# enkeejunior1/Diffusion-Pullback

Measured on AMD Instinct MI355X. Metric: pullback top-k SVD iters/sec (SD-v1.5 mid-block, 4x64x64), higher is better.
Workload: dtype bf16; 1 GPU; BASELINE configs[2]: SD-v1.5 4x64x64 latent, no edit prompt (seeded null ctx[1,77,768]), mid-block h[1280,8,8], t=696.27; pca_rank=5, ctx=null, samples_total=5, samples_this_rank=5, samples_advanced_together=1, spectrum=shaped (configs.Spectrum()), parallelism=single process, no collective, rccl_world_size=0, repeats=7

## Files before the change

diffusion_pullback_amd/csrc/engine.cpp:

```cpp
#include <math.h>
#include <stdarg.h>
#include <stdio.h>
#include <stdlib.h>
#include <string.h>

#include <string>
#include <vector>

#include "../../include/dpb.h"
#include "kernels.h"

namespace dpb {

static thread_local char g_err[1024] = "";
void set_error(const char* fmt, ...) {
  va_list ap;
  va_start(ap, fmt);
  vsnprintf(g_err, sizeof(g_err), fmt, ap);
  va_end(ap);
}
const char* last_error() { return g_err; }

static inline size_t align_up(size_t v, size_t a = 256) { return (v + a - 1) / a * a; }
static inline int round8(int v) { return (v + 7) / 8 * 8; }
// ... 1077 lines not shown
  int n = b.kind == DPB_BUF_SHARED ? 1 : e->cur_batch;
  if (n < 1) return fail("no primal state to read (dpb_forward invalidates it; run dpb_primal first)");
  return launch_nhwc_to_nchw(e->dtype, e->P(buf), out, n, channels, b.rows, b.C, e->stream);
}

static int jvp_pass(dpb_engine* e, int src, int tap, const float* V, int nt, float* U) {
  if (!e || !V) return fail("null argument");
  if (int r = check_pair(e, src, tap, nt)) return r;
  e->n_launch = 0; e->flops = 0; e->gbytes = 0;
  const Buf& bx = e->bufs[src];
  e->n_launch++;
  if (int r = launch_nchw_to_nhwc(e->dtype, V, e->T(src), nt, seed_channels(e, src), bx.rows, bx.C, e->stream)) return r;
  if (e->tstats_bytes && !gn_deterministic()) DPB_CHECK(hipMemsetAsync(e->ws + e->tstats_off, 0, e->tstats_bytes, e->stream));
  const int last = e->producer[tap];
  std::fill(e->skip.begin(), e->skip.end(), 0);
  e->cur_tap = tap; e->pend.on = false;
  for (int i = e->producer[src] + 1; i <= last; ++i) {
    if (!e->oact[i] || e->skip[i]) continue;
    if (int r = run_op(e, e->ops[i], MODE_TANGENT, nt)) return r;
  }
  if (int r = flush_pending(e)) return r;
  if (!U) return 0;
  const Buf& bt = e->bufs[tap];
  e->n_launch++;
  return launch_nhwc_to_nchw(e->dtype, e->T(tap), U, nt, bt.Cv, bt.rows, bt.C, e->stream);
}

int dpb_jvp(dpb_engine* e, int tap, const float* V, int nt, float* U) {
  if (!U) return fail("null argument");
  return jvp_pass(e, e ? e->x_buf : -1, tap, V, nt, U);
}

int dpb_jvp_between(dpb_engine* e, int src_buf, int dst_buf, const float* V, int nt, float* U) {
  if (!e || !U) return fail("null argument");
  return jvp_pass(e, src_buf, dst_buf, V, nt, U);
}

static int vjp_pass(dpb_engine* e, int src, int tap, const float* U, int nt, float* W) {
  if (!e || !W) return fail("null argument");
  if (int r = check_pair(e, src, tap, nt)) return r;
  e->n_launch = 0; e->flops = 0; e->gbytes = 0;
  const Buf& bt = e->bufs[tap];
  std::fill(e->ginit.begin(), e->ginit.end(), 0);
  for (auto& b : e->bufs) b.g_off = b.g_off0;
  if (U) {
    e->n_launch++;
    if (int r = launch_nchw_to_nhwc(e->dtype, U, e->G(tap), nt, bt.Cv, bt.rows, bt.C, e->stream)) return r;
  } else {
    e->bufs[tap].g_off = e->bufs[tap].t_off;
  }
  e->ginit[tap] = 1;
  if (e->tstats_bytes && !gn_deterministic()) DPB_CHECK(hipMemsetAsync(e->ws + e->tstats_off, 0, e->tstats_bytes, e->stream));
  e->cur_tap = tap; e->pend.on = false;
  for (int i = e->producer[tap]; i > e->producer[src]; --i) {
    const Op& op = e->ops[i];
    if (!e->oact[i] || !e->ginit[op.d.out]) continue;
    if (int r = run_op(e, op, MODE_ADJOINT, nt)) return r;
  }
  if (int r = flush_pending(e)) return r;
  if (!e->ginit[src]) {
    for (auto& b : e->bufs) b.g_off = b.g_off0;
    return src == e->x_buf ? fail("tap buffer %d is not connected to x", tap) : fail("dst buffer %d is not connected to source buffer %d", tap, src);
  }
  const Buf& bx = e->bufs[src];
  e->n_launch++;
  const int r = launch_nhwc_to_nchw(e->dtype, e->G(src), W, nt, seed_channels(e, src), bx.rows, bx.C, e->stream);
  for (auto& b : e->bufs) b.g_off = b.g_off0;
  return r;
}

int dpb_vjp(dpb_engine* e, int tap, const float* U, int nt, float* W) {
  if (!U) return fail("null argument");
  return vjp_pass(e, e ? e->x_buf : -1, tap, U, nt, W);
}

int dpb_vjp_between(dpb_engine* e, int src_buf, int dst_buf, const float* U, int nt, float* W) {
  if (!e || !U) return fail("null argument");
  return vjp_pass(e, src_buf, dst_buf, U, nt, W);
}

int dpb_orth(const float* W, const float* Vprev, float* V, float* s, float* conv, void* scratch, int k, int64_t N, void* stream) {
  if (!W || !Vprev || !V || !s || !conv || !scratch) return fail("null argument");
  OrthArgs a;
  a.W = W; a.Vprev = Vprev; a.V = V; a.s = s; a.conv = conv; a.scratch = (double*)scratch; a.k = k; a.N = N;
  a.scratch_bytes = orth_scratch_bytes(k, N);
  return launch_orth(a, (hipStream_t)stream);
}

int dpb_orth_checked(const float* W, const float* Vprev, float* V, float* s, float* conv, void* scratch, size_t scratch_bytes, int k, int64_t N,
                     void* stream) {
  if (!W || !Vprev || !V || !s || !conv || !scratch) return fail("null argument");
  if (k < 1 || k > ORTH_MAX_RANK || N < 1) return fail("dpb_orth: k=%d outside [1,%d] or N=%lld < 1", k, ORTH_MAX_RANK, (long long)N);
  const size_t need = orth_scratch_bytes(k, N);
  if (scratch_bytes < need) return fail("dpb_orth: scratch of %zu bytes, dpb_orth_scratch_bytes(%d, %lld) = %zu", scratch_bytes, k, (long long)N, need);
  OrthArgs a;
  a.W = W; a.Vprev = Vprev; a.V = V; a.s = s; a.conv = conv; a.scratch = (double*)scratch; a.k = k; a.N = N;
  a.scratch_bytes = scratch_bytes;
  return launch_orth(a, (hipStream_t)stream);
}

size_t dpb_orth_scratch_bytes(int k, int64_t N) { return (k < 1 || k > ORTH_MAX_RANK || N < 1) ? 0 : orth_scratch_bytes(k, N); }

size_t dpb_pca_scratch_bytes(int q, int64_t N, int64_t D) { return pca_scratch_bytes(q, N, D); }

int dpb_pca_lowrank(const float* H, int64_t N, int64_t D, const float* R, int q, int niter, float* u, float* s, void* scratch,
                    size_t scratch_bytes, void* stream) {
  if (!H || !R || !u || !s || (!scratch && scratch_bytes)) return fail("dpb_pca_lowrank: null argument");
  return launch_pca_lowrank(H, N, D, R, q, niter, u, s, scratch, scratch_bytes, (hipStream_t)stream);
}

static int g_iter_alias = getenv("DPB_ITER_ALIAS") ? atoi(getenv("DPB_ITER_ALIAS")) : 1;
static int g_orth_batch = getenv("DPB_ORTH_BATCH") ? atoi(getenv("DPB_ORTH_BATCH")) : 1;
static int g_graph_iterate = 0;

static int iterate_pass(dpb_engine* e, int src, int tap, float* V, float* U, float* s, float* conv, int k, int n_iters, float* Wm, char* orth_scratch,
                        size_t orth_stride) {
  const int B = e->cur_batch;
  const int nt = k * B;
  const long N = (long)e->bufs[src].rows * seed_channels(e, src);
  long launches = 0; double fl = 0, gb = 0;
  const bool alias_ok = e->bufs[tap].Cv == e->bufs[tap].C && g_iter_alias;
  auto body = [&](bool want_u) -> int {
    const bool keep = alias_ok && !want_u;
    if (int r = jvp_pass(e, src, tap, V, nt, keep ? nullptr : U)) return r;
    launches += e->n_launch; fl += e->flops; gb += e->gbytes;
    if (int r = vjp_pass(e, src, tap, keep ? nullptr : U, nt, Wm)) return r;
    launches += e->n_launch; fl += e->flops; gb += e->gbytes;
    {
      OrthArgs a;
      a.W = Wm; a.Vprev = V; a.V = V; a.s = s; a.conv = conv; a.scratch = (double*)orth_scratch; a.k = k; a.N = N;
      a.scratch_bytes = orth_scratch_bytes(k, N);
      a.batch = B; a.stride_w = (long)k * N; a.stride_v = (long)k * N; a.stride_s = k; a.stride_conv = 2; a.scratch_stride = orth_stride;
      if (g_orth_batch) {
        if (int r = launch_orth(a, e->stream)) return r;
      } else {
        a.batch = 1;
        for (int b = 0; b < B; ++b) {
          if (int r = launch_orth(a, e->stream)) return r;
          a.W += a.stride_w; a.Vprev += a.stride_v; a.V += a.stride_v; a.s += k; a.conv += 2; a.scratch += orth_stride / sizeof(double);
        }
      }
    }
    launches += g_orth_batch ? 4 : 4 * B;
    return 0;
  };
  int it = 0;
  if (g_graph_iterate && !e->profiling && e->stream != 0 && src == e->x_buf) {
    const dpb_engine::GraphKey key{tap, k, B, V, U, s, conv};
    if (!e->gexec || !(key == e->gkey)) {
      if (int r = body(true)) return r;
      ++it;
      if (e->gexec) { (void)hipGraphExecDestroy(e->gexec); e->gexec = nullptr; }
      hipGraph_t g = nullptr;
      const long l0 = launches; const double f0 = fl, b0 = gb;
      DPB_CHECK(hipStreamBeginCapture(e->stream, hipStreamCaptureModeThreadLocal));
      const int r = body(true);
      const hipError_t ce = hipStreamEndCapture(e->stream, &g);
      e->g_launches = launches - l0; e->g_flops = fl - f0; e->g_bytes = gb - b0;
      launches = l0; fl = f0; gb = b0;
      if (r) { if (g) (void)hipGraphDestroy(g); return r; }
      DPB_CHECK(ce);
      DPB_CHECK(hipGraphInstantiate(&e->gexec, g, nullptr, nullptr, 0));
      (void)hipGraphDestroy(g);
      e->gkey = key;
    }
    for (; it < n_iters; ++it) {
      DPB_CHECK(hipGraphLaunch(e->gexec, e->stream));
      launches += e->g_launches; fl += e->g_flops; gb += e->g_bytes;
    }
  }
  for (; it < n_iters; ++it)
    if (int r = body(it == n_iters - 1)) return r;
  e->n_launch = launches; e->flops = fl; e->gbytes = gb;
  return 0;
}

int dpb_pullback_iterate(dpb_engine* e, int tap, float* V, float* U, float* s, float* conv, int k, int n_iters) {
  if (!e || !V || !U || !s || !conv) return fail("null argument");
  if (k < 1 || k > ORTH_MAX_RANK) return fail("pca_rank k=%d outside [1,%d]", k, ORTH_MAX_RANK);
  const int B = e->cur_batch;
  if (int r = check_tap(e, tap, k * (B > 0 ? B : 1))) return r;
  return iterate_pass(e, e->x_buf, tap, V, U, s, conv, k, n_iters, (float*)(e->ws + e->pbW), e->ws + e->orth, e->orth_stride);
}

static size_t between_scratch_bytes(const dpb_engine* e, int src, int k, int batch) {
  const long N = (long)e->bufs[src].rows * seed_channels(e, src);
  return align_up((size_t)batch * k * N * sizeof(float)) + (size_t)batch * align_up(orth_scratch_bytes(k, N));
}

size_t dpb_pullback_scratch_bytes(const dpb_engine* e, int src_buf, int k) {
  if (!e || k < 1 || k > ORTH_MAX_RANK || src_buf < 0 || src_buf >= (int)e->bufs.size() || e->bufs[src_buf].kind != DPB_BUF_ACT) return 0;
  return between_scratch_bytes(e, src_buf, k, e->maxB);
}

int dpb_pullback_iterate_between(dpb_engine* e, int src_buf, int dst_buf, float* V, float* U, float* s, float* conv, int k, int n_iters, void* scratch,
                                 size_t scratch_bytes) {
  if (!e || !V || !U || !s || !conv || !scratch) return fail("null argument");
  if (k < 1 || k > ORTH_MAX_RANK) return fail("pca_rank k=%d outside [1,%d]", k, ORTH_MAX_RANK);
  const int B = e->cur_batch;
  if (int r = check_pair(e, src_buf, dst_buf, k * (B > 0 ? B : 1))) return r;
  if ((uintptr_t)scratch % 256) return fail("scratch must be 256-byte aligned");
  const size_t need = between_scratch_bytes(e, src_buf, k, B);
  if (scratch_bytes < need) return fail("scratch of %zu bytes, the iteration needs %zu (dpb_pullback_scratch_bytes)", scratch_bytes, need);
  const long N = (long)e->bufs[src_buf].rows * seed_channels(e, src_buf);
  const size_t wbytes = align_up((size_t)B * k * N * sizeof(float));
  return iterate_pass(e, src_buf, dst_buf, V, U, s, conv, k, n_iters, (float*)scratch, (char*)scratch + wbytes, align_up(orth_scratch_bytes(k, N)));
}

int dpb_ddim_step(const float* x, const float* eps, float* out, float* x0, int64_t n, float a_t, float a_next, void* stream) {
  if (!x || !eps || !out) return fail("null argument");
  return launch_ddim_step(x, eps, out, x0, n, a_t, a_next, (hipStream_t)stream);
}

int dpb_embed_tokens(const int32_t* ids, const void* tok_table, const void* pos_table, int dtype, float* out, int batch, int tokens,
                     int channels, int vocab, void* stream) {
  if (!ids || !tok_table || !pos_table || !out) return fail("null argument");
  if (dtype != DPB_F32 && dtype != DPB_BF16 && dtype != DPB_F16) return fail("bad dtype %d", dtype);
  return launch_embed_tokens(dtype, ids, tok_table, pos_table, out, batch, tokens, channels, vocab, (hipStream_t)stream);
}

int dpb_lincomb(const float* x, const float* y, const float* z, float* out, int64_t n, float a, float b, float c, void* stream) {
  if (!x || !y || !out) return fail("null argument");
  return launch_lincomb(x, y, z, out, n, a, b, c, (hipStream_t)stream);
}

int dpb_engine_profile(dpb_engine* e, int enable) {
  if (!e) return fail("null engine");
  for (auto& p : e->prof) { (void)hipEventDestroy(p.a); (void)hipEventDestroy(p.b); }
  e->prof.clear();
  e->profiling = enable != 0;
  if (e->profiling) {
    hipEvent_t a, b;
    DPB_CHECK(hipEventCreate(&a));
    DPB_CHECK(hipEventCreate(&b));
    float best = 1e9f;
    for (int i = 0; i < 24; ++i) {
      DPB_CHECK(hipEventRecord(a, e->stream));
      if (int r = launch_axpy(e->dtype, e->ws + e->zeros, e->ws + e->zeros, 64, 0, e->stream)) return r;
      DPB_CHECK(hipEventRecord(b, e->stream));
      DPB_CHECK(hipEventSynchronize(b));
      float ms = 0;
      DPB_CHECK(hipEventElapsedTime(&ms, a, b));
      if (i >= 4) best = ms < best ? ms : best;
    }
    (void)hipEventDestroy(a);
    (void)hipEventDestroy(b);
    best -= 1.5e-3f;
    if (best < 0.f) best = 0.f;
    e->prof_overhead_ms = best < 1e8f ? best : 0.f;
  }
  return 0;
}

int dpb_engine_profile_dump(dpb_engine* e, const char* path) {
  if (!e || !path) return fail("null argument");
  DPB_CHECK(hipStreamSynchronize(e->stream));
  FILE* f = fopen(path, "w");
  if (!f) return fail("cannot open %s", path);
  fprintf(f, "idx,big,gather,M,N,K,Z,us,tflops,raw_us,bracket_overhead_us\n");
  int i = 0;
  for (auto& p : e->prof) {
    float raw = 0;
    (void)hipEventElapsedTime(&raw, p.a, p.b);
    const float ms = raw > e->prof_overhead_ms ? raw - e->prof_overhead_ms : 0.f;
    fprintf(f, "%d,%d,%d,%d,%d,%d,%d,%.2f,%.2f,%.2f,%.2f\n", i++, p.big, p.gather, p.M, p.N, p.K, p.Z, ms * 1e3, ms > 0 ? p.flops / (ms * 1e-3) / 1e12 : 0.0,
            raw * 1e3, e->prof_overhead_ms * 1e3);
  }
  fclose(f);
  return 0;
}

int dpb_engine_profile_read(dpb_engine* e, int big_tile, int64_t* count, double* total_ms, double* flops) {
  if (!e || !count || !total_ms || !flops) return fail("null argument");
  DPB_CHECK(hipStreamSynchronize(e->stream));
  *count = 0; *total_ms = 0; *flops = 0;
  const bool raw = big_tile >= 1000;
  if (raw) big_tile -= 1000;
  if (big_tile < 0 || big_tile > 12) return fail("dpb_engine_profile_read: kind must be 0..12 or 1000..1012");
  for (auto& p : e->prof) {
    if (p.big != big_tile) continue;
    float ms = 0;
    DPB_CHECK(hipEventElapsedTime(&ms, p.a, p.b));
    if (!raw) ms = ms > e->prof_overhead_ms ? ms - e->prof_overhead_ms : 0.f;
    *count += 1; *total_ms += ms; *flops += p.flops;
  }
  return 0;
}

int dpb_engine_profile_overhead(const dpb_engine* e, double* bracket_overhead_ms) {
  if (!e || !bracket_overhead_ms) return fail("null argument");
  *bracket_overhead_ms = e->prof_overhead_ms;
  return 0;
}

int dpb_debug_set(const char* key, int value) {
  static int tile = 0, splitk = 0, kch = 0;
  if (!key) return fail("null key");
  if (!strcmp(key, "gemm_tile")) tile = value;
  else if (!strcmp(key, "gemm_splitk")) splitk = value;
  else if (!strcmp(key, "gemm_kch")) kch = value;
  else if (!strcmp(key, "gemm_dma_auto")) { gemm_debug_dma_auto(value); return 0; }
  else if (!strcmp(key, "gemm_order")) { gemm_debug_order(value); return 0; }
  else if (!strcmp(key, "p8")) { gemm_debug_p8(value); return 0; }
  else if (!strcmp(key, "wres")) { gemm_debug_wres(value); return 0; }
  else if (!strcmp(key, "gn_deterministic")) { gn_debug_deterministic(value); return 0; }
  else if (!strcmp(key, "graph_iterate")) { g_graph_iterate = value; return 0; }
  else if (!strcmp(key, "attn_shared")) { attn_debug_shared(value); return 0; }
  else if (!strcmp(key, "lazy_reduce")) { g_lazy_reduce = value; return 0; }
  else if (!strcmp(key, "ln_fuse")) { g_ln_fuse = value; return 0; }
  else if (!strcmp(key, "cross_primal")) { g_cross_primal = value; return 0; }
  else if (!strcmp(key, "geglu_fwd")) { g_geglu_fwd = value; return 0; }
  else if (!strcmp(key, "iter_alias")) { g_iter_alias = value; return 0; }
  else return fail("unknown debug key %s", key);
  gemm_debug_set(tile, splitk, kch);
  return 0;
}

int dpb_debug_gemm_plan(int dtype, int M, int N, int K, int conv_hw, int conv_cin, int epilogue, int64_t slab_bytes, int* kind, int* tile,
                        int* splitk) {
  if (!kind || !tile || !splitk) return fail("null argument");
  if (dtype != DPB_F32 && dtype != DPB_BF16 && dtype != DPB_F16) return fail("bad dtype %d", dtype);
  static char dummy[16];
  GemmArgs a;
  a.M = M; a.N = N; a.K = K; a.lda = K; a.ldb = K; a.ldc = N;
  a.zeros = dummy;
  if (slab_bytes > 0) { a.slab = (float*)dummy; a.slab_bytes = (size_t)slab_bytes; }
  a.epi = epilogue;
  if (conv_hw > 0) {
    if (conv_cin <= 0 || K != 9 * conv_cin || M % (conv_hw * conv_hw)) return fail("conv plan: K must be 9*cin and M whole images");
    a.gather = GATHER_CONV; a.H = a.W = a.Ho = a.Wo = conv_hw; a.Cin = conv_cin; a.KS = 3; a.stride = 1; a.pad = 1; a.lda = conv_cin;
  }
  const GemmPlan pl = gemm_plan(dtype, a);
  if (pl.kind < 0) return -1;
  *kind = pl.kind; *tile = pl.tile; *splitk = pl.splitk;
  return 0;
}

int dpb_engine_stats(const dpb_engine* e, int64_t* launches, double* gemm_flops, double* gemm_bytes) {
  if (!e) return fail("null engine");
  if (launches) *launches = e->n_launch;
  if (gemm_flops) *gemm_flops = e->flops;
  if (gemm_bytes) *gemm_bytes = e->gbytes;
  return 0;
}

}
```

diffusion_pullback_amd/csrc/gemm_halo.hip:

```cpp
#include "epilogue.h"

namespace dpb {

typedef __attribute__((address_space(3))) void lds_void_t;
typedef __attribute__((address_space(1))) const void gbl_void_t;

__device__ inline bf16x8 halo_lds_read(unsigned addr) {
  bf16x8 v;
  asm volatile("ds_read_b128 %0, %1" : "=v"(v) : "v"(addr));
  return v;
}
__device__ inline void halo_wait_frags4(bf16x8 (&a)[2], bf16x8 (&b)[2]) {
  asm volatile("s_waitcnt lgkmcnt(4)" : "+v"(a[0]), "+v"(a[1]), "+v"(b[0]), "+v"(b[1]));
}
__device__ inline void halo_wait_frags0(bf16x8 (&a)[2], bf16x8 (&b)[2]) {
  asm volatile("s_waitcnt lgkmcnt(0)" : "+v"(a[0]), "+v"(a[1]), "+v"(b[0]), "+v"(b[1]));
}
__device__ inline void halo_wait_vm(int n) {
  if (n >= 13) asm volatile("s_waitcnt vmcnt(13)" ::: "memory");
  else if (n == 11) asm volatile("s_waitcnt vmcnt(11)" ::: "memory");
  else if (n == 9) asm volatile("s_waitcnt vmcnt(9)" ::: "memory");
  else if (n == 7) asm volatile("s_waitcnt vmcnt(7)" ::: "memory");
  else if (n == 4) asm volatile("s_waitcnt vmcnt(4)" ::: "memory");
  else if (n == 2) asm volatile("s_waitcnt vmcnt(2)" ::: "memory");
  else asm volatile("s_waitcnt vmcnt(0)" ::: "memory");
}

constexpr int HALO_BM = 256, HALO_BN = 128, HALO_NH = 7;
constexpr int HALO_MAXPIX = 400;
constexpr int HALO_BYTES = ((HALO_MAXPIX * 8 + 63) / 64) * 1024;
constexpr int HALO_BSTAGE = HALO_BN * 128, HALO_S = 3;

template <int GATHER, int FL = 0>
__global__ __launch_bounds__(512) void conv_halo_kernel(GemmArgs p) {
  constexpr int BM = HALO_BM, BN = HALO_BN, WAVES = 8, NH = HALO_NH, S = HALO_S, KK = 4;
  constexpr int NIB = BN / (8 * WAVES);
  constexpr int WN = BN / 2, SLD = WN + 4;
  constexpr int B0 = 2 * HALO_BYTES, DUMMY = B0 + S * HALO_BSTAGE;
  constexpr int SMEM_BYTES = DUMMY + 1024;
  static_assert(SMEM_BYTES >= WAVES * 32 * SLD * 4 && SMEM_BYTES <= 160 * 1024, "LDS budget");
  __shared__ __attribute__((aligned(128))) char smem[SMEM_BYTES];
  const unsigned lds0 = (unsigned)(uintptr_t)(lds_void_t*)smem;

  const int tid = threadIdx.x, lane = tid & 63, wave = tid >> 6;
  const int tilesN = (p.N + BN - 1) / BN, tilesM = (p.M + BM - 1) / BM;
  int lin = blockIdx.x + gridDim.x * (blockIdx.y + gridDim.y * blockIdx.z);
  {
    const int nwg = gridDim.x * gridDim.y * gridDim.z, q = nwg >> 3, r = nwg & 7, xcd = lin & 7, idx = lin >> 3;
    lin = (xcd < r ? xcd * (q + 1) : r * (q + 1) + (xcd - r) * q) + idx;
  }
  int tm, tn;
  if (p.order == 0) { tn = lin % tilesN; lin /= tilesN; tm = lin % tilesM; lin /= tilesM; }
  else { tm = lin % tilesM; lin /= tilesM; tn = lin % tilesN; lin /= tilesN; }
  const int ksplit = lin;
  const int m0 = tm * BM, n0 = tn * BN;
  const bf16* A = (const bf16*)p.A;
  const bf16* B = (const bf16*)p.B;
  bf16* C = (bf16*)p.C;
  const bf16* R = (const bf16*)p.R;
  const bf16* zero = (const bf16*)p.zeros;

  const int W = p.W, H = p.H, Cin = p.Cin, lda = p.lda, HWp = W + 2;
  const int hw = H * W, SPT = hw >= BM ? 1 : BM / hw, RT = hw >= BM ? BM / W : H;
  const int smp = m0 / hw, y0 = hw >= BM ? (m0 - smp * hw) / W : 0, nsmp = p.M / hw;
  const int hpix = (RT + 2) * HWp, npix = SPT * hpix, tpix = RT * W;
  const int nch_all = Cin / 64;
  int c_begin = 0, nch = nch_all;
  if (p.splitk > 1) {
    const int per = (nch_all + p.splitk - 1) / p.splitk;
    c_begin = ksplit * per;
    nch = max(0, min(nch_all, c_begin + per) - c_begin);
  }
  const int ns = nch * 9;

  const bf16* h_src[NH];
  int h_dst[NH];
#pragma unroll
  for (int i = 0; i < NH; ++i) {
    const int inst = wave * NH + i, slot = inst * 64 + lane, pix = slot >> 3, phys = slot & 7;
    h_dst[i] = inst * 1024 < HALO_BYTES ? inst * 1024 : -1;
    h_src[i] = nullptr;
    if (pix < npix) {
      const int sl = pix / hpix, rp = pix - sl * hpix, hy = rp / HWp, hx = rp - hy * HWp, iy = y0 - 1 + hy, ix = hx - 1;
      if (smp + sl < nsmp && iy >= 0 && iy < H && ix >= 0 && ix < W)
        h_src[i] = A + ((long)((smp + sl) * H + iy) * W + ix) * lda + ((phys ^ ((pix >> 1) & 7)) << 3);
    }
  }
  const bf16* b_src[NIB];
#pragma unroll
  for (int i = 0; i < NIB; ++i) {
    const int pos = (wave * NIB + i) * 64 + lane, row = pos >> 3, phys = pos & 7, n = n0 + row;
    b_src[i] = n < p.N ? B + (long)n * p.ldb + ((phys ^ ((row >> 1) & 7)) << 3) : nullptr;
  }
  auto issue_halo = [&](int c) {
    char* hb = smem + (c & 1) * HALO_BYTES;
#pragma unroll
    for (int i = 0; i < NH; ++i) {
      const bf16* src = h_src[i] ? h_src[i] + c * 64 : zero;
      char* dst = h_dst[i] >= 0 ? hb + h_dst[i] : smem + DUMMY;
      __builtin_amdgcn_global_load_lds((gbl_void_t*)src, (lds_void_t*)dst, 16, 0, 0);
    }
  };
  auto issue_b = [&](int s) {
    const int c = c_begin + s / 9, tap = s - (s / 9) * 9;
    char* st = smem + B0 + (s % S) * HALO_BSTAGE;
    const int koff = tap * Cin + c * 64;
#pragma unroll
    for (int i = 0; i < NIB; ++i) {
      const bf16* src = b_src[i] ? b_src[i] + koff : zero;
      __builtin_amdgcn_global_load_lds((gbl_void_t*)src, (lds_void_t*)(st + (wave * NIB + i) * 1024), 16, 0, 0);
    }
  };

  f32x16 acc[2][2];
#pragma unroll
  for (int i = 0; i < 2; ++i)
#pragma unroll
    for (int j = 0; j < 2; ++j)
#pragma unroll
      for (int r = 0; r < 16; ++r) acc[i][j][r] = 0.f;

  const int wy = wave >> 1, wx = wave & 1, l31 = lane & 31, lhi = lane >> 5;
  int pixm[2];
#pragma unroll
  for (int i = 0; i < 2; ++i) {
    const int m = wy * 64 + i * 32 + l31, sl = m / tpix, r = m - sl * tpix, oy = r / W, ox = r - oy * W;
    pixm[i] = sl * hpix + (oy + 1) * HWp + ox + 1;
  }
  unsigned fb0[2];
#pragma unroll
  for (int j = 0; j < 2; ++j) {
    const int row = wx * WN + j * 32 + l31;
    fb0[j] = B0 + row * 128 + ((lhi ^ ((row >> 1) & 7)) << 4);
  }
  bf16x8 fa[2][2], fb[2][2];
  unsigned abase[2], asw[2];
  auto set_stage = [&](int s) {
    const int c = c_begin + s / 9, tap = s - (s / 9) * 9, ky = (tap * 11) >> 5, kx = tap - ky * 3;
    const int toff = GATHER == GATHER_CONV ? (ky - 1) * HWp + (kx - 1) : (1 - ky) * HWp + (1 - kx);
#pragma unroll
    for (int i = 0; i < 2; ++i) {
      const int pix = pixm[i] + toff;
      abase[i] = lds0 + (c & 1) * HALO_BYTES + pix * 128;
      asw[i] = (pix >> 1) & 7;
    }
  };
  auto read_frags = [&](int s, int kk, int buf) {
    const unsigned sbB = lds0 + (s % S) * HALO_BSTAGE;
#pragma unroll
    for (int i = 0; i < 2; ++i) fa[buf][i] = halo_lds_read(abase[i] + ((((kk << 1) | lhi) ^ asw[i]) << 4));
#pragma unroll
    for (int j = 0; j < 2; ++j) fb[buf][j] = halo_lds_read(sbB + (fb0[j] ^ (kk << 5)));
  };

  if (ns > 0) {
    issue_halo(c_begin);
    issue_b(0);
    if (ns > 1) issue_b(1);
    if (nch > 1) issue_halo(c_begin + 1);
    if (ns > 2) issue_b(2);
    halo_wait_vm((ns > 1 ? 2 : 0) + (nch > 1 ? NH : 0) + (ns > 2 ? 2 : 0));
    __builtin_amdgcn_s_barrier();
    set_stage(0);
    read_frags(0, 0, 0);
    for (int s = 0; s < ns; ++s) {
#pragma unroll
      for (int kk = 0; kk < KK; ++kk) {
        const int cur = kk & 1, nxt = cur ^ 1;
        if (kk + 1 < KK) {
          read_frags(s, kk + 1, nxt);
          halo_wait_frags4(fa[cur], fb[cur]);
        } else {
          halo_wait_frags0(fa[cur], fb[cur]);
          if (s + 1 < ns) {
            const int tap_s = s - (s / 9) * 9, ch_s = s / 9;
            halo_wait_vm((s + 2 < ns ? 2 : 0) + ((tap_s == 0 && ch_s + 1 < nch) ? NH : 0));
            __builtin_amdgcn_s_barrier();
            const int tap_n = tap_s == 8 ? 0 : tap_s + 1, ch_n = tap_s == 8 ? ch_s + 1 : ch_s;
            if (tap_n == 0 && ch_n + 1 < nch) issue_halo(c_begin + ch_n + 1);
            if (s + 3 < ns) issue_b(s + 3);
            set_stage(s + 1);
            read_frags(s + 1, 0, nxt);
          }
        }
        __builtin_amdgcn_sched_barrier(0);
#pragma unroll
        for (int i = 0; i < 2; ++i)
#pragma unroll
          for (int j = 0; j < 2; ++j) acc[i][j] = H16<FL>::mfma(fa[cur][i], fb[cur][j], acc[i][j]);
        __builtin_amdgcn_sched_barrier(0);
      }
    }
  }
  asm volatile("s_waitcnt vmcnt(0) lgkmcnt(0)" ::: "memory");
  __syncthreads();

  float* stage = reinterpret_cast<float*>(smem) + wave * 32 * SLD;
#pragma unroll
  for (int i = 0; i < 2; ++i) {
#pragma unroll
    for (int j = 0; j < 2; ++j)
#pragma unroll
      for (int r = 0; r < 16; ++r) stage[((r & 3) + 8 * (r >> 2) + 4 * lhi) * SLD + j * 32 + l31] = acc[i][j][r];
    __syncthreads();
    epilogue_slab<FL, WN, SLD, EPI_PLAIN>(p, C, R, reinterpret_cast<const float*>(smem), wave, lane, m0 + wy * 64 + i * 32, n0, (long)ksplit);
    __syncthreads();
  }
}

int conv_halo_supported(const GemmArgs& a) {
  if (a.gather != GATHER_CONV && a.gather != GATHER_CONVT) return 0;
  if (a.KS != 3 || a.stride != 1 || a.pad != 1 || a.Z1 * a.Z2 != 1 || a.A2) return 0;
  if (a.H != a.Ho || a.W != a.Wo || a.Cin % 64 || a.K != 9 * a.Cin) return 0;
  const int hw = a.H * a.W;
  if (a.M % hw) return 0;
  if (hw >= HALO_BM) {
    if (HALO_BM % a.W || hw % HALO_BM) return 0;
    if ((HALO_BM / a.W + 2) * (a.W + 2) > HALO_MAXPIX) return 0;
  } else {
    if (HALO_BM % hw || a.W < 8) return 0;
    if ((HALO_BM / hw) * (a.H + 2) * (a.W + 2) > HALO_MAXPIX) return 0;
  }
  if (a.lda % 8 || a.ldb % 8 || !a.zeros) return 0;
  return 1;
}

int launch_conv_halo(const GemmArgs& a, hipStream_t st) {
  const int sk = a.splitk > 1 ? a.splitk : 1;
  dim3 grid(((a.M + HALO_BM - 1) / HALO_BM) * ((a.N + HALO_BN - 1) / HALO_BN), 1, sk);
  if (a.gather == GATHER_CONV) {
    if (a.fl) hipLaunchKernelGGL((conv_halo_kernel<GATHER_CONV, 1>), grid, dim3(512), 0, st, a);
    else hipLaunchKernelGGL((conv_halo_kernel<GATHER_CONV, 0>), grid, dim3(512), 0, st, a);
  } else {
    if (a.fl) hipLaunchKernelGGL((conv_halo_kernel<GATHER_CONVT, 1>), grid, dim3(512), 0, st, a);
    else hipLaunchKernelGGL((conv_halo_kernel<GATHER_CONVT, 0>), grid, dim3(512), 0, st, a);
  }
  DPB_CHECK(hipGetLastError());
  return 0;
}

}
```

diffusion_pullback_amd/csrc/kernels.h:

```cpp
#pragma once
#include <algorithm>

#include "common.h"

namespace dpb {

enum { GATHER_NONE = 0, GATHER_CONV = 1, GATHER_CONVT = 2, GATHER_UPCONV = 3 };
enum { EPI_PLAIN = 0, EPI_GEGLU_TAN = 1, EPI_GEGLU_ADJ = 2, EPI_LN_TAN = 3, EPI_LN_ADJ = 4, EPI_GEGLU_FWD = 5 };
struct GemmArgs {
  const void* A = nullptr; const void* B = nullptr; void* C = nullptr; const void* R = nullptr;
  const float* bias = nullptr;
  const void* rowbias = nullptr;
  int rows_per_sample = 1, rowbias_div = 1;
  int M = 0, N = 0, K = 0;
  int lda = 0, ldb = 0, ldc = 0, ldr = 0;
  int Z1 = 1, Z2 = 1;
  long sA1 = 0, sA2 = 0, sB1 = 0, sB2 = 0, sC1 = 0, sC2 = 0, sR1 = 0, sR2 = 0;
  int divA = 1, divB = 1;
  float alpha = 1.f;
  int accumulate = 0;
  int gather = GATHER_NONE;
  int H = 0, W = 0, Cin = 0, Ho = 0, Wo = 0, KS = 1, stride = 1, pad = 0;
  const void* A2 = nullptr; const void* B2 = nullptr;
  int K2 = 0, lda2 = 0, ldb2 = 0, divA2 = 1, divB2 = 1;
  long sA21 = 0, sA22 = 0, sB21 = 0, sB22 = 0;
  float* slab = nullptr; size_t slab_bytes = 0;
  const void* zeros = nullptr;
  int splitk = 1, vec_ok = 0;
  int epi = EPI_PLAIN, epi_kps = 1;
  const void* hprim = nullptr;
  const void* ln_x = nullptr; const float* ln_gamma = nullptr; float ln_eps = 1e-5f; void* C2 = nullptr;
  int fl = 0;
  int order = 0;
};
struct GemmPlan { int kind, tile, splitk; };
int launch_gemm(int dtype, const GemmArgs& a, hipStream_t st, int* launches = nullptr, GemmArgs* pending = nullptr);
int launch_gemm_reduce(int dtype, const GemmArgs& pending, hipStream_t st);
GemmPlan gemm_plan(int dtype, const GemmArgs& a);
int gemm_uses_big_tile(int dtype, const GemmArgs& a);
void gemm_debug_set(int tile, int splitk, int kch);
int gemm_kch(const GemmArgs& a);
int launch_gemm_dma(const GemmArgs& a, int tile, hipStream_t st);
int launch_gemm_ring64(const GemmArgs& a, int tile, hipStream_t st);
bool gemm_p8_fits32(const GemmArgs& a);
int launch_gemm_p8(const GemmArgs& a, int tile, hipStream_t st);
int conv_halo_supported(const GemmArgs& a);
int launch_conv_halo(const GemmArgs& a, hipStream_t st);
int gemm_uses_halo(int dtype, const GemmArgs& a);
int gemm_epi_supported(int dtype, const GemmArgs& a);
int gemm_uses_dma(int dtype, const GemmArgs& a);
void gemm_debug_dma_auto(int on);
void gn_debug_deterministic(int on);
int gn_deterministic();
bool gemm_wres_supported(int dtype, const GemmArgs& a);
int launch_gemm_wres(const GemmArgs& a, hipStream_t st);
void gemm_debug_wres(int on);
void gemm_debug_p8(int on);
void gemm_debug_order(int o);
int gemm_pick_splitk_dma(const GemmArgs& a, int tile);

enum { MODE_PRIMAL = 0, MODE_TANGENT = 1, MODE_ADJOINT = 2 };
struct SlabSrc {
  const float* slab = nullptr; int splitk = 0; long MN = 0; int N = 0;
  const void* R = nullptr; int ldr = 0;
  void* store = nullptr;
};
struct GNArgs {
  const void* x = nullptr;
  const void* d = nullptr;
  void* y = nullptr;
  const float* gamma = nullptr; const float* beta = nullptr;
  double* pstats = nullptr;
  double* tstats = nullptr;
  float* part = nullptr;
  size_t part_bytes = 0;
  int* ticket = nullptr;
  int det = 1;
  int red = 0;
  int Bp = 1, NT = 0, kps = 1;
  int HW = 0, C = 0, G = 32;
  float eps = 1e-5f;
  int silu = 0, accumulate = 0;
  SlabSrc src;
};
int launch_groupnorm(int dtype, int mode, const GNArgs& a, hipStream_t st);
int groupnorm_launches(int dtype, int mode, const GNArgs& a);

struct LNArgs {
  const void* x = nullptr; const void* d = nullptr; void* y = nullptr;
  const float* gamma = nullptr; const float* beta = nullptr;
  int rows_per_sample = 0, Bp = 1, NT = 0, kps = 1, C = 0;
  float eps = 1e-5f;
  int accumulate = 0;
  SlabSrc src;
};
int launch_layernorm(int dtype, int mode, const LNArgs& a, hipStream_t st);

int launch_softmax_fwd(int dtype, void* S, long Z, int Lq, int Lk, int ld, int causal, hipStream_t st);
int launch_softmax_jvp(int dtype, const void* P, void* dS, float* D, long Z, int Z2, int kps, int Lq, int Lk, int ld,
                       hipStream_t st);
int launch_softmax_adjT(int dtype, const void* PT, void* gPT, const float* D, long Z, int Z2, int kps, int Lk, int Lq,
                        int ld, hipStream_t st);
int launch_transpose(int dtype, const void* in, void* out, int Z1, int Z2, long s1, long s2, int R, int Ccols, int ldin,
                     int ldout, long outZstride, hipStream_t st);

struct FusedAttnArgs {
  const void *Q = nullptr, *K = nullptr, *V = nullptr, *O = nullptr, *KT = nullptr, *VT = nullptr, *QT = nullptr;
  const float* stats = nullptr;
  float* Drow = nullptr;
  const void *dQ = nullptr, *dK = nullptr, *dV = nullptr, *dVT = nullptr; void* dO = nullptr;
  const void *gO = nullptr, *gOT = nullptr; void *gQ = nullptr, *gK = nullptr, *gV = nullptr;
  int accQ = 0, accK = 0, accV = 0;
  int fl = 0;
  int L = 0, C = 0, Co = 0, H = 0, d = 0, kps = 1;
  float scale = 1.f;
};
int fused_attention_supported(int dtype, int d, int L, int kv_const);
void attn_debug_shared(int bits);
struct CrossAttnArgs {
  const void *Q = nullptr, *K = nullptr, *V = nullptr;
  const void* BT = nullptr;
  const void* X = nullptr; void* Y = nullptr;
  int L = 0, Lk = 0, Lkp = 0, C = 0, Ck = 0, Cx = 0, Cy = 0, H = 0, d = 0, kps = 1, adjoint = 0, accumulate = 0, fl = 0;
  int primal = 0;
  float scale = 1.f;
};
int cross_attention_supported(int dtype, int d, int Lq, int Lk, int kv_const);
int launch_attn_cross(const CrossAttnArgs& f, int nt, hipStream_t st);
int launch_row_stats(int fl, const void* S, float* stats, long nrows, int Lk, int ld, hipStream_t st);
int attn_adj_route_bits(int d, int L, int kps, int nt);
int attn_adj_launches(int d, int L, int kps, int nt);
int attn_jvp_block_waves(int d, int L, int pairs);
int launch_attn_fwd_fused(const FusedAttnArgs& f, int batch, void* O, float* stats, hipStream_t st);
int launch_attn_jvp_fused(const FusedAttnArgs& f, int nt, hipStream_t st);
int launch_attn_adj_fused(const FusedAttnArgs& f, int nt, hipStream_t st);

struct GegluArgs {
  const void* h = nullptr;
  const void* d = nullptr;
  void* y = nullptr;
  int rows_per_sample = 0, Bp = 1, NT = 0, kps = 1, F = 0;
  int accumulate = 0;
  int stash = 1;
  int il = 0;
};
int launch_geglu(int dtype, int mode, const GegluArgs& a, hipStream_t st);
int launch_silu(int dtype, const void* x, void* y, long n, hipStream_t st);
int launch_quick_gelu(int dtype, const void* x, void* y, long n, hipStream_t st);
int launch_gelu(int dtype, const void* x, void* y, long n, hipStream_t st);
int launch_embed_tokens(int dtype, const int* ids, const void* tok, const void* pos, float* out, int batch, int L, int C, int vocab, hipStream_t st);
int launch_axpy(int dtype, const void* x, void* y, long n, int accumulate, hipStream_t st);
int launch_copy_cols(int dtype, const void* src, int lds, int cs0, void* dst, int ldd, int cd0, long rows, int ncols,
                     int accumulate, hipStream_t st);
int launch_zero_cols(int dtype, void* dst, int ldd, int cd0, long rows, int ncols, hipStream_t st);
int launch_nchw_to_nhwc(int dtype, const float* src, void* dst, int n, int C, int HW, int Cpad, hipStream_t st);
int launch_nhwc_to_nchw(int dtype, const void* src, float* dst, int n, int C, int HW, int Cpad, hipStream_t st);
int launch_pool2x2_sum(int dtype, const void* in, void* out, int n, int H, int W, int C, int accumulate, hipStream_t st);

struct OrthArgs {
  const float* W = nullptr;
  const float* Vprev = nullptr;
  float* V = nullptr;
  float* s = nullptr;
  float* conv = nullptr;
  double* scratch = nullptr;
  size_t scratch_bytes = 0;
  int k = 0; long N = 0;
  int batch = 1; long stride_w = 0, stride_v = 0, stride_s = 0, stride_conv = 0; size_t scratch_stride = 0;
};
constexpr int ORTH_MAX_RANK = 128;
int launch_orth(const OrthArgs& a, hipStream_t st);
size_t orth_scratch_bytes(int k, long N);

const char* pca_invalid(int q, long N, long D);
size_t pca_scratch_bytes(int q, long N, long D);
int launch_pca_lowrank(const float* H, long N, long D, const float* R, int q, int niter, float* u, float* s, void* scratch, size_t scratch_bytes,
                       hipStream_t st);

int launch_ddim_step(const float* x, const float* e, float* out, float* x0, long n, float a_t, float a_next, hipStream_t st);
int launch_lincomb(const float* x, const float* y, const float* z, float* out, long n, float a, float b, float c, hipStream_t st);

}
```

Baseline: 117.7 iters/s.

## Add phased 8-wave software-pipelined main loop for halo conv kernel

```diff
diff --git a/diffusion_pullback_amd/csrc/engine.cpp b/diffusion_pullback_amd/csrc/engine.cpp
--- a/diffusion_pullback_amd/csrc/engine.cpp
+++ b/diffusion_pullback_amd/csrc/engine.cpp
@@ -1403,6 +1403,7 @@
   else if (!strcmp(key, "gemm_dma_auto")) { gemm_debug_dma_auto(value); return 0; }
   else if (!strcmp(key, "gemm_order")) { gemm_debug_order(value); return 0; }
   else if (!strcmp(key, "p8")) { gemm_debug_p8(value); return 0; }
+  else if (!strcmp(key, "halo_loop")) { conv_halo_debug_loop(value); return 0; }
   else if (!strcmp(key, "wres")) { gemm_debug_wres(value); return 0; }
   else if (!strcmp(key, "gn_deterministic")) { gn_debug_deterministic(value); return 0; }
   else if (!strcmp(key, "graph_iterate")) { g_graph_iterate = value; return 0; }
diff --git a/diffusion_pullback_amd/csrc/gemm_halo.hip b/diffusion_pullback_amd/csrc/gemm_halo.hip
--- a/diffusion_pullback_amd/csrc/gemm_halo.hip
+++ b/diffusion_pullback_amd/csrc/gemm_halo.hip
@@ -30,16 +30,16 @@
 constexpr int HALO_MAXPIX = 400;
 constexpr int HALO_BYTES = ((HALO_MAXPIX * 8 + 63) / 64) * 1024;
 constexpr int HALO_BSTAGE = HALO_BN * 128, HALO_S = 3;
-
-template <int GATHER, int FL = 0>
-__global__ __launch_bounds__(512) void conv_halo_kernel(GemmArgs p) {
+constexpr int HALO_SMEM = 2 * HALO_BYTES + HALO_S * HALO_BSTAGE + 1024;
+
+template <int GATHER, int FL>
+__device__ __forceinline__ void halo_ring_loop(const GemmArgs& p, char* smem) {
   constexpr int BM = HALO_BM, BN = HALO_BN, WAVES = 8, NH = HALO_NH, S = HALO_S, KK = 4;
   constexpr int NIB = BN / (8 * WAVES);
   constexpr int WN = BN / 2, SLD = WN + 4;
   constexpr int B0 = 2 * HALO_BYTES, DUMMY = B0 + S * HALO_BSTAGE;
   constexpr int SMEM_BYTES = DUMMY + 1024;
-  static_assert(SMEM_BYTES >= WAVES * 32 * SLD * 4 && SMEM_BYTES <= 160 * 1024, "LDS budget");
-  __shared__ __attribute__((aligned(128))) char smem[SMEM_BYTES];
+  static_assert(SMEM_BYTES >= WAVES * 32 * SLD * 4 && SMEM_BYTES <= HALO_SMEM, "LDS budget");
   const unsigned lds0 = (unsigned)(uintptr_t)(lds_void_t*)smem;
 
   const int tid = threadIdx.x, lane = tid & 63, wave = tid >> 6;
@@ -208,6 +208,219 @@
   }
 }
 
+template <int OFF>
+__device__ __forceinline__ bf16x8 halo_read_at(unsigned addr) {
+  bf16x8 v;
+  asm volatile("ds_read_b128 %0, %1 offset:%2" : "=v"(v) : "v"(addr), "n"(OFF));
+  return v;
+}
+__device__ __forceinline__ void halo_wait12(bf16x8 (&a)[2][4], bf16x8 (&b)[4]) {
+  asm volatile("s_waitcnt lgkmcnt(0)"
+               : "+v"(a[0][0]), "+v"(a[0][1]), "+v"(a[0][2]), "+v"(a[0][3]), "+v"(a[1][0]), "+v"(a[1][1]), "+v"(a[1][2]), "+v"(a[1][3]), "+v"(b[0]), "+v"(b[1]),
+                 "+v"(b[2]), "+v"(b[3]));
+}
+__device__ __forceinline__ void halo_wait4(bf16x8 (&b)[4]) {
+  asm volatile("s_waitcnt lgkmcnt(0)" : "+v"(b[0]), "+v"(b[1]), "+v"(b[2]), "+v"(b[3]));
+}
+
+constexpr int HP8_PH = 18, HP8_LOOK = 4, HP8_SLOTS = 6, HP8_HALF = 64 * 128;
+constexpr int hp8_vm(int j) {
+  int n = HP8_LOOK - 1;
+  for (int t = j - (HP8_LOOK - 2); t <= j; ++t) n += (t >= 0 && t < HALO_NH);
+  return n;
+}
+
+template <int GATHER, int FL>
+__device__ __forceinline__ void halo_p8_loop(const GemmArgs& p, char* smem) {
+  constexpr int BM = HALO_BM, BN = HALO_BN, NH = HALO_NH, PH = HP8_PH, LOOK = HP8_LOOK, NSLOT = HP8_SLOTS, HALF = HP8_HALF;
+  constexpr int WN = BN / 2, SLD = WN + 4;
+  constexpr int B0 = 2 * HALO_BYTES, SINK = B0 + NSLOT * HALF;
+  static_assert(SINK + 1024 <= HALO_SMEM && 8 * 32 * SLD * 4 <= HALO_SMEM, "LDS budget");
+  static_assert(HALF == 8 * 1024 && BN == 128, "a half tile = 64 columns x 64 channels = one 1 KiB DMA instruction per wave");
+  static_assert(NSLOT >= LOOK + 2 && PH % NSLOT == 0 && PH % 2 == 0, "WAR: a slot is restaged >= 2 phases after its read; static slots per chunk");
+  static_assert(NH <= PH - LOOK + 1 && NH <= 7, "the halo of chunk c+1 is covered by the waits of chunk c");
+  static_assert(hp8_vm(0) == 4 && hp8_vm(2) == 6 && hp8_vm(7) == 5 && hp8_vm(9) == 3, "the counted waits of the header");
+  static_assert((NSLOT - 1) * HALF < 65536, "slot offsets are ds_read immediates");
+  const unsigned lds0 = (unsigned)(uintptr_t)(lds_void_t*)smem;
+
+  const int tid = threadIdx.x, lane = tid & 63;
+  const int wave = __builtin_amdgcn_readfirstlane(tid >> 6);
+  const int tilesN = (p.N + BN - 1) / BN, tilesM = (p.M + BM - 1) / BM;
+  int lin = blockIdx.x + gridDim.x * (blockIdx.y + gridDim.y * blockIdx.z);
+  {
+    const int nwg = gridDim.x * gridDim.y * gridDim.z, q = nwg >> 3, r = nwg & 7, xcd = lin & 7, idx = lin >> 3;
+    lin = (xcd < r ? xcd * (q + 1) : r * (q + 1) + (xcd - r) * q) + idx;
+  }
+  int tm, tn;
+  if (p.order == 0) { tn = lin % tilesN; lin /= tilesN; tm = lin % tilesM; lin /= tilesM; }
+  else { tm = lin % tilesM; lin /= tilesM; tn = lin % tilesN; lin /= tilesN; }
+  const int ksplit = lin;
+  const int m0 = tm * BM, n0 = tn * BN;
+  const bf16* A = (const bf16*)p.A;
+  const bf16* B = (const bf16*)p.B;
+  bf16* C = (bf16*)p.C;
+  const bf16* R = (const bf16*)p.R;
+  const bf16* zero = (const bf16*)p.zeros;
+
+  const int W = p.W, H = p.H, Cin = p.Cin, lda = p.lda, HWp = W + 2;
+  const int hw = H * W, SPT = hw >= BM ? 1 : BM / hw, RT = hw >= BM ? BM / W : H;
+  const int smp = m0 / hw, y0 = hw >= BM ? (m0 - smp * hw) / W : 0, nsmp = p.M / hw;
+  const int hpix = (RT + 2) * HWp, npix = SPT * hpix, tpix = RT * W;
+  const int nch_all = Cin / 64;
+  int c_begin = 0, nch = nch_all;
+  if (p.splitk > 1) {
+    const int per = (nch_all + p.splitk - 1) / p.splitk;
+    c_begin = ksplit * per;
+    nch = max(0, min(nch_all, c_begin + per) - c_begin);
+  }
+
+  const bf16* h_src[NH];
+  int h_dst[NH];
+#pragma unroll
+  for (int i = 0; i < NH; ++i) {
+    const int inst = wave * NH + i, slot = inst * 64 + lane, pix = slot >> 3, phys = slot & 7;
+    h_dst[i] = inst * 1024 < HALO_BYTES ? inst * 1024 : -1;
+    h_src[i] = nullptr;
+    if (pix < npix) {
+      const int sl = pix / hpix, rp = pix - sl * hpix, hy = rp / HWp, hx = rp - hy * HWp, iy = y0 - 1 + hy, ix = hx - 1;
+      if (smp + sl < nsmp && iy >= 0 && iy < H && ix >= 0 && ix < W)
+        h_src[i] = A + ((long)((smp + sl) * H + iy) * W + ix) * lda + ((phys ^ ((pix >> 1) & 7)) << 3);
+    }
+  }
+  const bf16* b_src[2];
+#pragma unroll
+  for (int h = 0; h < 2; ++h) {
+    const int pos = wave * 64 + lane, r = pos >> 3, phys = pos & 7, n = n0 + (r >> 5) * 64 + h * 32 + (r & 31);
+    b_src[h] = n < p.N ? B + (long)n * p.ldb + ((phys ^ ((r >> 1) & 7)) << 3) : nullptr;
+  }
+  auto issue_halo = [&](auto ic, int c) {
+    constexpr int i = decltype(ic)::value;
+    const bf16* src = (h_src[i] && c < nch) ? h_src[i] + (c_begin + c) * 64 : zero;
+    char* dst = h_dst[i] >= 0 ? smem + (c & 1) * HALO_BYTES + h_dst[i] : smem + SINK;
+    __builtin_amdgcn_global_load_lds((gbl_void_t*)src, (lds_void_t*)dst, 16, 0, 0);
+  };
+  auto issue_b = [&](auto jc, int c) {
+    constexpr int j = decltype(jc)::value, h = j & 1, tap = j >> 1, slot = j % NSLOT;
+    const bf16* src = (b_src[h] && c < nch) ? b_src[h] + tap * Cin + (c_begin + c) * 64 : zero;
+    __builtin_amdgcn_global_load_lds((gbl_void_t*)src, (lds_void_t*)(smem + B0 + slot * HALF + wave * 1024), 16, 0, 0);
+  };
+
+  f32x16 acc[2][2];
+#pragma unroll
+  for (int i = 0; i < 2; ++i)
+#pragma unroll
+    for (int j = 0; j < 2; ++j)
+#pragma unroll
+      for (int r = 0; r < 16; ++r) acc[i][j][r] = 0.f;
+
+  const int wy = wave >> 1, wx = wave & 1, l31 = lane & 31, lhi = lane >> 5;
+  int pixm[2];
+#pragma unroll
+  for (int i = 0; i < 2; ++i) {
+    const int m = wy * 64 + i * 32 + l31, sl = m / tpix, r = m - sl * tpix, oy = r / W, ox = r - oy * W;
+    pixm[i] = sl * hpix + (oy + 1) * HWp + ox + 1;
+  }
+  unsigned adB[4];
+#pragma unroll
+  for (int kk = 0; kk < 4; ++kk) {
+    const int r = wx * 32 + l31;
+    adB[kk] = lds0 + B0 + r * 128 + ((((kk << 1) | lhi) ^ ((r >> 1) & 7)) << 4);
+  }
+  bf16x8 fa[2][4], fb0[4], fb1[4];
+  auto read_a = [&](auto tc, int c) {
+    constexpr int tap = decltype(tc)::value, ky = tap / 3, kx = tap % 3;
+    const int toff = GATHER == GATHER_CONV ? (ky - 1) * HWp + (kx - 1) : (1 - ky) * HWp + (1 - kx);
+    const unsigned hb = lds0 + (c & 1) * HALO_BYTES;
+#pragma unroll
+    for (int i = 0; i < 2; ++i) {
+      int pc = pixm[i];
+      asm volatile("" : "+v"(pc));
+      const int pix = pc + toff, sw = (pix >> 1) & 7;
+#pragma unroll
+      for (int kk = 0; kk < 4; ++kk) fa[i][kk] = halo_lds_read(hb + pix * 128 + ((((kk << 1) | lhi) ^ sw) << 4));
+    }
+  };
+  auto read_b = [&](auto sc, bf16x8 (&fb)[4]) {
+    constexpr int o = decltype(sc)::value * HALF;
+#pragma unroll
+    for (int kk = 0; kk < 4; ++kk) fb[kk] = halo_read_at<o>(adB[kk]);
+  };
+  auto mma = [&](auto hc, bf16x8 (&fb)[4]) {
+    constexpr int h = decltype(hc)::value;
+    __builtin_amdgcn_sched_barrier(0);
+    __builtin_amdgcn_s_setprio(1);
+#pragma unroll
+    for (int kk = 0; kk < 4; ++kk) {
+      acc[0][h] = H16<FL>::mfma(fa[0][kk], fb[kk], acc[0][h]);
+      acc[1][h] = H16<FL>::mfma(fa[1][kk], fb[kk], acc[1][h]);
+    }
+    __builtin_amdgcn_s_setprio(0);
+    __builtin_amdgcn_sched_barrier(0);
+  };
+  auto bar = [&]() {
+    __builtin_amdgcn_sched_barrier(0);
+    __builtin_amdgcn_s_barrier();
+    __builtin_amdgcn_sched_barrier(0);
+  };
+  using I0 = std::integral_constant<int, 0>;
+  using I1 = std::integral_constant<int, 1>;
+
+  auto phase = [&](auto jc, int c) {
+    constexpr int j = decltype(jc)::value, tap = j >> 1, h = j & 1, jn = j + LOOK;
+    using SLOT = std::integral_constant<int, j % NSLOT>;
+    if constexpr (h == 0) {
+      read_a(std::integral_constant<int, tap>{}, c);
+      read_b(SLOT{}, fb0);
+    } else {
+      read_b(SLOT{}, fb1);
+    }
+    if constexpr (j < NH) issue_halo(jc, c + 1);
+    if constexpr (jn < PH) issue_b(std::integral_constant<int, jn>{}, c);
+    else issue_b(std::integral_constant<int, jn - PH>{}, c + 1);
+    asm volatile("s_waitcnt vmcnt(%0)" ::"n"(hp8_vm(j)) : "memory");
+    bar();
+    if constexpr (h == 0) {
+      halo_wait12(fa, fb0);
+      mma(I0{}, fb0);
+    } else {
+      halo_wait4(fb1);
+      mma(I1{}, fb1);
+    }
+    bar();
+  };
+
+  if (nch > 0) {
+    static_for<0, NH>([&](auto ic) { issue_halo(ic, 0); });
+    static_for<0, LOOK>([&](auto jc) { issue_b(jc, 0); });
+    asm volatile("s_waitcnt vmcnt(%0)" ::"n"(LOOK - 1) : "memory");
+    bar();
+    if (wave >= 4) bar();
+    for (int c = 0; c < nch; ++c) static_for<0, PH>([&](auto jc) { phase(jc, c); });
+    if (wave < 4) bar();
+  }
+  asm volatile("s_waitcnt vmcnt(0) lgkmcnt(0)" ::: "memory");
+  __syncthreads();
+
+  float* stage = reinterpret_cast<float*>(smem) + wave * 32 * SLD;
+#pragma unroll
+  for (int i = 0; i < 2; ++i) {
+#pragma unroll
+    for (int j = 0; j < 2; ++j)
+#pragma unroll
+      for (int r = 0; r < 16; ++r) stage[((r & 3) + 8 * (r >> 2) + 4 * lhi) * SLD + j * 32 + l31] = acc[i][j][r];
+    __syncthreads();
+    epilogue_slab<FL, WN, SLD, EPI_PLAIN>(p, C, R, reinterpret_cast<const float*>(smem), wave, lane, m0 + wy * 64 + i * 32, n0, (long)ksplit);
+    __syncthreads();
+  }
+}
+
+template <int GATHER, int FL, int LOOP>
+__global__ __launch_bounds__(512) void conv_halo_kernel(GemmArgs p) {
+  __shared__ __attribute__((aligned(1024))) char smem[HALO_SMEM];
+  if constexpr (LOOP) halo_p8_loop<GATHER, FL>(p, smem);
+  else halo_ring_loop<GATHER, FL>(p, smem);
+}
+
 int conv_halo_supported(const GemmArgs& a) {
   if (a.gather != GATHER_CONV && a.gather != GATHER_CONVT) return 0;
   if (a.KS != 3 || a.stride != 1 || a.pad != 1 || a.Z1 * a.Z2 != 1 || a.A2) return 0;
@@ -225,15 +438,25 @@
   return 1;
 }
 
+static int g_halo_loop = 1;
+void conv_halo_debug_loop(int on) { g_halo_loop = on; }
+
+template <int GATHER, int FL>
+static void launch_halo_g(const GemmArgs& a, dim3 grid, hipStream_t st) {
+  static const int loop_env = getenv("DPB_HALO_LOOP") ? atoi(getenv("DPB_HALO_LOOP")) : 1;
+  if (loop_env && g_halo_loop) hipLaunchKernelGGL((conv_halo_kernel<GATHER, FL, 1>), grid, dim3(512), 0, st, a);
+  else hipLaunchKernelGGL((conv_halo_kernel<GATHER, FL, 0>), grid, dim3(512), 0, st, a);
+}
+
 int launch_conv_halo(const GemmArgs& a, hipStream_t st) {
   const int sk = a.splitk > 1 ? a.splitk : 1;
   dim3 grid(((a.M + HALO_BM - 1) / HALO_BM) * ((a.N + HALO_BN - 1) / HALO_BN), 1, sk);
   if (a.gather == GATHER_CONV) {
-    if (a.fl) hipLaunchKernelGGL((conv_halo_kernel<GATHER_CONV, 1>), grid, dim3(512), 0, st, a);
-    else hipLaunchKernelGGL((conv_halo_kernel<GATHER_CONV, 0>), grid, dim3(512), 0, st, a);
+    if (a.fl) launch_halo_g<GATHER_CONV, 1>(a, grid, st);
+    else launch_halo_g<GATHER_CONV, 0>(a, grid, st);
   } else {
-    if (a.fl) hipLaunchKernelGGL((conv_halo_kernel<GATHER_CONVT, 1>), grid, dim3(512), 0, st, a);
-    else hipLaunchKernelGGL((conv_halo_kernel<GATHER_CONVT, 0>), grid, dim3(512), 0, st, a);
+    if (a.fl) launch_halo_g<GATHER_CONVT, 1>(a, grid, st);
+    else launch_halo_g<GATHER_CONVT, 0>(a, grid, st);
   }
   DPB_CHECK(hipGetLastError());
   return 0;
diff --git a/diffusion_pullback_amd/csrc/kernels.h b/diffusion_pullback_amd/csrc/kernels.h
--- a/diffusion_pullback_amd/csrc/kernels.h
+++ b/diffusion_pullback_amd/csrc/kernels.h
@@ -46,6 +46,7 @@
 int launch_gemm_p8(const GemmArgs& a, int tile, hipStream_t st);
 int conv_halo_supported(const GemmArgs& a);
 int launch_conv_halo(const GemmArgs& a, hipStream_t st);
+void conv_halo_debug_loop(int on);
 int gemm_uses_halo(int dtype, const GemmArgs& a);
 int gemm_epi_supported(int dtype, const GemmArgs& a);
 int gemm_uses_dma(int dtype, const GemmArgs& a);
```

Result: faster. 119.9 iters/s, median of 6 (+1.9%).
